# mako443/Text2Pos-CVPR2022

Hardware: AMD Instinct MI355X
Metric: cells+queries encoded/sec and top-k retrieval QPS, 256-pt cells, 12k-cell DB (higher is better)
Workload: dtype f16x3 (fp32 operands split hi+lo into fp16, 3 f16 MFMAs, fp32 accumulate; fp32-class error) for the encoders / f64 MFMA for the ranking

## Files before the change

text2pos-cvpr2022_amd/csrc/cell_encoder.hip:

```cpp
#include "../../include/t2p.h"
#include "t2p_common.h"

namespace t2p {
namespace {

struct Geo {
    int nd[3], nc[3];
    int gp;
    static constexpr int H[3] = {32, 128, 256};
    static constexpr int C[3] = {64, 128, 256};
    static constexpr int LD[3] = {96, 160, 288};
    explicit Geo(int n_pts) {
        nd[0] = n_pts;
        for (int l = 0; l < 3; l++) {
            nc[l] = (nd[l] + 1) / 2;
            if (l < 2) nd[l + 1] = nc[l];
        }
        gp = 1;
        while (gp < nc[2]) gp *= 2;
    }
    bool specialised(int l) const {
        static constexpr int ND[3] = {256, 128, 64}, NC[3] = {128, 64, 32};
        return nd[l] == ND[l] && nc[l] == NC[l];
    }
// ... 194 lines not shown
        T2P_TRY(launch_build_rows(xyz, rgb, n, cfg.n_pts, cfg.radius, gt, st));
    else if (prune_l0)
        T2P_TRY(launch_dedup_rows(xyz, rgb, n, cfg.n_pts, gt.rows[0], gt.n_rows[0], g.nc[0], st));
    return launch_sa_balance_levels(bp, Geo::H, Geo::C, st);
}

int Chunk::sa_levels(const float* xyz, const float* rgb) const {
    for (int l = 0; l < 3; l++) {
        const int H = Geo::H[l], C = Geo::C[l];
        const int cf = l == 0 ? 3 : Geo::C[l - 1];
        if (l != 0) {
            WsParams p{};
            p.A = ws.F[l - 1];
            p.lda = Geo::LD[l - 1];
            p.k_live = Geo::C[l - 1] + 4;
            p.W = W.sa_w1[l];
            p.W_x3 = f16x3() ? W.sa_w1_x3[l] : nullptr;
            p.ldw = H;
            p.bias = W.sa_b1[l];
            p.out = ws.A[l];
            p.ldo = H;
            p.relu = 0;
            p.M = n * g.nd[l];
            p.amax_out = gslot(l == 1 ? G_A2 : G_A3);
            T2P_TRY(launch_ws(WS_DENSE_STORE, Geo::LD[l - 1] - (f16x3() ? 16 : 0), H, p, st));
        }
        SaParams p{};
        p.A = ws.A[l];
        p.Bc = ws.B[l];
        p.wp = lds_btab(l) ? W.sa_w1[l] + (size_t)cf * Geo::H[l] : nullptr;
        p.W = W.sa_w2[l];
        p.W_x3 = f16x3() ? W.sa_w2_x3[l] : nullptr;
        p.bias = f16x3() ? W.sa_b2_x3[l] : W.sa_b2[l];
        p.out_scale = f16x3() ? 1.0f / W.sa_w2_scale[l] : 1.0f;
        p.out = ws.F[l];
        p.ldo = Geo::LD[l];
        p.rows = ws.gt.rows[l];
        p.n_rows = ws.gt.n_rows[l];
        p.first = ws.first;
        p.fps_idx = ws.gt.fps_idx[l];
        p.pos_src = l == 0 ? xyz : ws.F[l - 1];
        p.ld_pos = l == 0 ? 3 : Geo::LD[l - 1];
        p.pos_col0 = l == 0 ? 0 : Geo::C[l - 1];
        if (l == 0 && sa1_points()) {
            p.feat_src = rgb;
            p.w1 = W.sa_w1[0];
            p.b1 = W.sa_b1[0];
        }
        p.n_dense = g.nd[l];
        p.n_cent = g.nc[l];
        p.n_obj = n;
        p.prefix_ws = ws.prefix[l];
        p.bounds_ws = ws.bounds[l];
        p.balanced = 1;
        p.amax_out = gslot(G_F1 + l);
        if (l == 2) p.out_rows = g.gp;
        T2P_TRY(launch_ws_sa(H, C, p, st));
    }
    return 0;
}

int Chunk::global_abstraction() const {
    WsParams p{};
    p.A = ws.F[2];
    p.lda = Geo::LD[2];
    p.W = W.ga_w1;
    p.W_x3 = f16x3() ? W.ga_w1_x3 : nullptr;
    p.ldw = 512;
    p.bias = W.ga_b1;
    p.out = ws.gh;
    _Float16* gh_hi = (_Float16*)ws.gh;
    _Float16* gh_lo = gh_hi + (size_t)gh_rows(n, g) * 512;
    if (f16x3()) {
        p.out_hi = gh_hi;
        p.out_lo = gh_lo;
        p.amax_out = gslot(G_GA_H);
    }
    p.ldo = 512;
    p.relu = 1;
    p.M = n * g.gp;
    T2P_TRY(launch_ws(WS_DENSE_STORE, Geo::LD[2] - (f16x3() ? 16 : 0), 512, p, st));
    WsParams q{};
    q.A = ws.gh;
    if (f16x3()) {
        q.A_hi = gh_hi;
        q.A_lo = gh_lo;
    }
    q.lda = 512;
    q.W = W.ga_w2;
    q.W_x3 = f16x3() ? W.ga_w2_x3 : nullptr;
    q.ldw = 1024;
    q.bias = W.ga_b2;
    q.out = ws.f0;
    q.ldo = 1024;
    q.relu = 1;
    q.M = n * g.gp;
    q.group_rows = g.gp;
    return launch_ws(WS_DENSE_GROUPMAX, 512, 1024, q, st);
}

int Chunk::trunk_heads() const {
    const bool x3 = f16x3() && W.lin1_x3 && W.lin2_x3;
    const DenseW lin1{W.lin1_w, x3 ? W.lin1_x3 : nullptr, W.lin1_scale}, lin2{W.lin2_w, x3 ? W.lin2_x3 : nullptr, W.lin2_scale};
    T2P_TRY(launch_dense(ws.f0, 1024, lin1, W.lin1_b, ws.f1, 512, 0, n, 1024, 512, 1, st, nullptr, 0, gslot(G_PN_F0)));
    return launch_dense(ws.f1, 512, lin2, W.lin2_b, ws.f2, 256, 0, n, 512, 256, 1, st, nullptr, 0, gslot(G_PN_F1));
}

int Chunk::trunk(const float* xyz, const float* rgb, bool want_nbr) const {
    T2P_TRY(group(xyz, rgb, want_nbr));
    T2P_TRY(sa_levels(xyz, rgb));
    T2P_TRY(global_abstraction());
    return trunk_heads();
}

int Chunk::object_encoder(const float* center, const float* mean_rgb, int32_t o_lo, const float** emb_out) const {
    const int D = cfg.embed_dim, nfeat = n_features(cfg), ldcat = nfeat * D;
    int slot = 0;
    if (cfg.use_class && cfg.class_embed) {
        T2P_TRY(launch_gather_rownorm(W.class_embedding, cfg.class_idx + o_lo, n, D, ws.cat, ldcat, slot * D, st));
        slot++;
    } else if (cfg.use_class) {
        const float* fin = cfg.pointnet_features == 0 ? ws.f0 : (cfg.pointnet_features == 1 ? ws.f1 : ws.f2);
        const int kin = cfg.pointnet_features == 0 ? 1024 : (cfg.pointnet_features == 1 ? 512 : 256);
        const DenseW pn{W.pn_w, f16x3() ? W.pn_x3 : nullptr, W.pn_scale};
        T2P_TRY(launch_dense(fin, kin, pn, W.pn_b, ws.P, D, 0, n, kin, D, 1, st, nullptr, 0, gslot(G_PN_F0 + cfg.pointnet_features)));
        T2P_TRY(launch_rownorm(ws.P, D, n, D, ws.cat, ldcat, slot * D, st));
        slot++;
    }
    if (cfg.use_color && cfg.color_embed) {
        T2P_TRY(launch_gather_rownorm(W.color_embedding, cfg.color_idx + o_lo, n, D, ws.cat, ldcat, slot * D, st));
        slot++;
    } else if (cfg.use_color) {
        T2P_TRY(launch_mlp3_norm(mean_rgb, n, W.col_w1, W.col_b1, W.col_w2, W.col_b2, D, ws.cat, ldcat, slot * D, st));
        slot++;
    }
    if (cfg.use_position) {
        T2P_TRY(launch_mlp3_norm(center, n, W.pos_w1, W.pos_b1, W.pos_w2, W.pos_b2, D, ws.cat, ldcat, slot * D, st));
        slot++;
    }
    *emb_out = ws.cat;
    if (nfeat > 1) {
        const DenseW merge{W.merge_w, f16x3() ? W.merge_x3 : nullptr, W.merge_scale};
        T2P_TRY(launch_dense(ws.cat, ldcat, merge, W.merge_b, ws.emb, D, 0, n, ldcat, D, 1, st, nullptr, 0, gslot(G_GEMM_IN)));
        *emb_out = ws.emb;
    }
    return 0;
}

int Chunk::cell_head(const float* emb, int max_cell, float* out) const {
    const int D = cfg.embed_dim;
    T2P_TRY(launch_rownorm(emb, D, n, D, ws.embn, D, 0, st));
    const bool x3 = f16x3() && W.g_wp_x3 && W.g_wq_x3;
    const DenseW wp{W.g_wp, x3 ? W.g_wp_x3 : nullptr, W.g_wp_scale}, wq{W.g_wq, x3 ? W.g_wq_x3 : nullptr, W.g_wq_scale};
    T2P_TRY(launch_dense(ws.embn, D, wp, W.g_bp, ws.P, D, 0, n, D, D, 0, st, nullptr, 0, gslot(G_GEMM_IN)));
    T2P_TRY(launch_dense(ws.embn, D, wq, nullptr, ws.Q, D, 0, n, D, D, 0, st, nullptr, 0, gslot(G_GEMM_IN)));
    T2P_TRY(launch_knn(ws.embn, D, ws.seg_ptr, (int)nb, max_cell, cfg.knn_k, ws.knn, st));
    WsParams p{};
    p.A = ws.Q;
    p.lda = D;
    p.Bc = ws.P;
    p.W = W.g_w2;
    p.W_x3 = f16x3() ? W.g_w2_x3 : nullptr;
    p.amax_out = gslot(G_EDGE);
    p.ldw = D;
    p.bias = W.g_b2;
    p.out = ws.x1;
    p.ldo = D;
    p.relu = 1;
    p.knn_group = (n + 31) / 32 < num_cus() ? 8 : 32;
    p.n_groups = (n + p.knn_group - 1) / p.knn_group;
    p.knn_idx = ws.knn;
    p.knn_k = cfg.knn_k;
    p.n_dst = n;
    p.mean = cfg.variation == 1;
    T2P_TRY(launch_ws(WS_EDGE_KNN, D, D, p, st));
    T2P_TRY(launch_segmax(ws.x1, D, ws.seg_ptr, (int)nb, ws.pool, cfg.variation == 1, st));
    T2P_TRY(launch_gemm(ws.pool, D, W.lin_w1, W.lin_b1, ws.l1, D, 0, nb, D, D, 1, st));
    T2P_TRY(launch_gemm(ws.l1, D, W.lin_w2, W.lin_b2, ws.l2, D, 0, nb, D, D, 1, st));
    return launch_rownorm(ws.l2, D, nb, D, out, D, 0, st);
}

template <typename T>
int copy_trace(T* dst, int64_t row0, size_t width, const T* src, int64_t n, hipStream_t st) {
    if (dst == nullptr || n == 0 || width == 0) return 0;
    hipError_t e = hipMemcpyAsync(dst + row0 * width, src, (size_t)n * width * sizeof(T), hipMemcpyDeviceToDevice, st);
    if (e != hipSuccess) {
        set_error("encode_cells: trace copy failed: %s", hipGetErrorString(e));
        return (int)e;
    }
    return 0;
}

int Chunk::copy_traces(const t2p_cell_trace& tr, int64_t obj0, bool trunk_ran, const float* emb) const {
    for (int l = 0; trunk_ran && l < 3; l++) {
        T2P_TRY(copy_trace(tr.fps_idx[l], obj0, g.nc[l], ws.gt.fps_idx[l], n, st));
        T2P_TRY(copy_trace(tr.nbr[l], obj0, (size_t)g.nc[l] * 32, ws.gt.nbr[l], n, st));
        T2P_TRY(copy_trace(tr.cnt[l], obj0, g.nc[l], ws.gt.cnt[l], n, st));
        if (tr.sa_out[l] && n > 0) {
            const int rows = l == 2 ? g.gp : g.nc[l];
            const size_t ld = Geo::LD[l] * sizeof(float);
            hipError_t e = hipSuccess;
            if (rows == g.nc[l])
                e = hipMemcpy2DAsync(tr.sa_out[l] + obj0 * g.nc[l] * Geo::LD[l], ld, ws.F[l], ld, (Geo::C[l] + 4) * sizeof(float),
                                     (size_t)n * g.nc[l], hipMemcpyDeviceToDevice, st);
            for (int cc = 0; rows != g.nc[l] && cc < g.nc[l] && e == hipSuccess; cc++)
                e = hipMemcpy2DAsync(tr.sa_out[l] + (obj0 * g.nc[l] + cc) * Geo::LD[l], g.nc[l] * ld, ws.F[l] + (size_t)cc * Geo::LD[l],
                                     rows * ld, (Geo::C[l] + 4) * sizeof(float), (size_t)n, hipMemcpyDeviceToDevice, st);
            if (e != hipSuccess) {
                set_error("encode_cells: trace copy failed: %s", hipGetErrorString(e));
                return (int)e;
            }
        }
    }
    if (trunk_ran) {
        T2P_TRY(copy_trace(tr.features0, obj0, 1024, ws.f0, n, st));
        T2P_TRY(copy_trace(tr.features1, obj0, 512, ws.f1, n, st));
        T2P_TRY(copy_trace(tr.features2, obj0, 256, ws.f2, n, st));
    }
    if (emb != nullptr) {
        T2P_TRY(copy_trace(tr.obj_emb, obj0, cfg.embed_dim, emb, n, st));
        T2P_TRY(copy_trace(tr.knn_idx, obj0, cfg.knn_k, ws.knn, n, st));
    }
    return 0;
}

int64_t next_chunk_end(const int32_t* cp, int64_t c0, int64_t n_cells, int chunk) {
    int64_t c1 = c0 + 1;
    while (c1 < n_cells && (cp[c1 + 1] - cp[c0]) <= chunk) c1++;
    return c1;
}

int fill_group_tables(const char* what, GroupTables& gt, int n_pts, int self_loops, int share_mask, uint8_t* const* fps_idx,
                      uint16_t* const* rows, uint16_t* const* n_rows, uint8_t* const* nbr, uint8_t* const* cnt) {
    const Geo g(n_pts);
    gt = GroupTables{};
    gt.self_loops = self_loops ? 1 : 0;
    for (int l = 0; l < 3; l++) {
        if (rows) T2P_CHECK_ARG(fps_idx[l] && rows[l] && n_rows[l], "%s: NULL table of level %d", what, l);
        gt.fps_idx[l] = fps_idx[l];
        gt.rows[l] = rows ? rows[l] : nullptr;
        gt.n_rows[l] = rows ? n_rows[l] : nullptr;
        gt.nbr[l] = nbr ? nbr[l] : nullptr;
        gt.cnt[l] = cnt ? cnt[l] : nullptr;
        gt.n_dense[l] = g.nd[l];
        gt.n_cent[l] = g.nc[l];
        gt.share_tail[l] = (share_mask >> l) & 1;
    }
    return 0;
}

int group_rows(const char* what, const float* xyz, int64_t n_obj, int32_t n_pts, const float* radius_host, int32_t self_loops,
               int32_t share_mask, uint8_t* const* fps_idx, uint16_t* const* rows, uint16_t* const* n_rows, t2p_stream_t stream) {
    T2P_CHECK_ARG(xyz && radius_host && fps_idx && rows && n_rows, "%s: NULL argument", what);
    T2P_CHECK_ARG((share_mask & ~2) == 0, "%s: share_mask=%#x (bit 1: SA level 2; no other level has a shared form)", what, share_mask);
    T2P_CHECK_ARG(share_mask == 0 || n_pts == 256, "%s: shared lists exist for 256 points per object (n_pts = %d)", what, n_pts);
    GroupTables gt;
    T2P_TRY(fill_group_tables(what, gt, n_pts, self_loops, share_mask, fps_idx, rows, n_rows, nullptr, nullptr));
    return launch_sample_group(xyz, n_obj, n_pts, radius_host, gt, (hipStream_t)stream);
}

int group_rows_built(const char* what, const float* xyz, const float* rgb, int64_t n_obj, int32_t n_pts, const float* radius_host,
                     int32_t self_loops, int32_t share_mask, int prune_dup, uint8_t* const* fps_idx, uint16_t* const* rows,
                     uint16_t* const* n_rows, t2p_stream_t stream) {
    T2P_CHECK_ARG(xyz && rgb && radius_host && fps_idx && rows && n_rows, "%s: NULL argument", what);
    T2P_CHECK_ARG(n_obj >= 0, "%s: negative size", what);
    T2P_CHECK_ARG((share_mask & ~2) == 0, "%s: share_mask=%#x (bit 1: SA level 2; no other level has a shared form)", what, share_mask);
    T2P_CHECK_ARG(n_pts == 256, "%s: built for 256 points per object (n_pts = %d)", what, n_pts);
    GroupTables gt;
    T2P_TRY(fill_group_tables(what, gt, n_pts, self_loops, share_mask, fps_idx, rows, n_rows, nullptr, nullptr));
    gt.mask_l0 = 1;
    gt.prune_dup[1] = gt.prune_dup[2] = prune_dup;
    T2P_CHECK_ARG((((uintptr_t)xyz | (uintptr_t)rgb | (uintptr_t)rows[0] | (uintptr_t)rows[1] | (uintptr_t)rows[2]) & 15) == 0,
                  "%s: xyz, rgb and rows must be 16-byte aligned", what);
    T2P_TRY(launch_sample_group(xyz, n_obj, n_pts, radius_host, gt, (hipStream_t)stream));
    return launch_build_rows(xyz, rgb, n_obj, n_pts, radius_host, gt, (hipStream_t)stream);
}

}
}

using namespace t2p;

extern "C" {

size_t t2p_encode_cells_workspace_bytes(int64_t n_obj, int64_t n_cells, const t2p_cell_config* cfg) {
    if (cfg == nullptr || n_obj <= 0) return 256;
    int64_t n = default_chunk(*cfg);
    if (n > n_obj) n = n_obj;
    int64_t nb = n_cells < n ? n_cells : n;
    Bump b{nullptr, 0, 0};
    return carve_cells(b, n, nb > 0 ? nb : 1, *cfg, nullptr) + 256;
}

int t2p_encode_cells(const float* xyz, const float* rgb, const float* center, const float* mean_rgb,
                     const int32_t* cell_ptr_host, const int32_t* cell_ptr, int64_t n_obj, int64_t n_cells,
                     const t2p_cell_weights* w, const t2p_cell_config* cfg, float* out, const t2p_cell_trace* trace,
                     void* workspace, size_t workspace_bytes, t2p_stream_t stream) {
    hipStream_t st = (hipStream_t)stream;
    T2P_TRY(check_cfg(cfg));
    T2P_CHECK_ARG(w != nullptr && cell_ptr_host != nullptr && cell_ptr != nullptr, "encode_cells: NULL argument");
    T2P_CHECK_ARG(n_cells >= 0 && n_obj >= 0, "encode_cells: negative size");
    if (n_cells == 0) return 0;
    if (cfg->objects_only)
        T2P_CHECK_ARG(trace != nullptr && trace->obj_emb != nullptr, "encode_cells: objects_only needs trace->obj_emb");
    else
        T2P_CHECK_ARG(out != nullptr, "encode_cells: out is NULL");
    T2P_CHECK_ARG(!cfg->class_embed || w->class_embedding != nullptr, "encode_cells: class_embedding weights missing");
    T2P_CHECK_ARG(!cfg->color_embed || w->color_embedding != nullptr, "encode_cells: color_embedding weights missing");
// ... 140 lines not shown
```

text2pos-cvpr2022_amd/csrc/t2p_common.h:

```cpp
#pragma once
#include <hip/hip_runtime.h>
#include <stdint.h>
#include <stdio.h>

namespace t2p {

void set_error(const char* fmt, ...);

#define T2P_E_ARG (-1)
#define T2P_E_WORKSPACE (-2)
#define T2P_E_UNSUPPORTED (-3)

#define T2P_CHECK_ARG(cond, ...)                  \
    do {                                          \
        if (!(cond)) {                            \
            ::t2p::set_error(__VA_ARGS__);        \
            return T2P_E_ARG;                     \
        }                                         \
    } while (0)

#define T2P_CHECK_LAUNCH(name)                                                   \
    do {                                                                         \
        hipError_t e__ = hipGetLastError();                                      \
        if (e__ != hipSuccess) {                                                 \
// ... 39 lines not shown
    return lo;
}
__device__ __forceinline__ void lds_barrier() { asm volatile("s_waitcnt lgkmcnt(0)\n\ts_barrier" ::: "memory"); }
typedef double f64x4 __attribute__((ext_vector_type(4)));

int num_cus();
int matrix_wgs();
int reserve_lds(const void* kernel, size_t bytes, const char* what);

inline size_t align_up(size_t v, size_t a) { return (v + a - 1) / a * a; }
struct Bump {
    char* base;
    size_t off, cap;
    template <typename T>
    T* take(size_t n) {
        off = align_up(off, 256);
        T* p = (T*)(base ? base + off : nullptr);
        off += n * sizeof(T);
        return p;
    }
};

enum GuardSlot {
    G_INPUT = 0,
    G_A2 = 2, G_A3 = 4,
    G_F1 = 6, G_F2 = 7, G_F3 = 8,
    G_GEMM_IN = 9,
    G_GA_H = 10, G_PN_F0 = 11, G_PN_F1 = 12, G_PN_F2 = 13, G_EDGE = 14,
    G_SLOTS = 16
};
struct GuardBounds {
    float wp_l1[3];
    float a1_l1;
    float a1_bmax;
    float ga1_l1;
    float ga1_bmax;
};
constexpr float kGuardFloor = 16384.f;
constexpr float kGuardTiny = 0.0078125f;
#ifdef __HIPCC__
__device__ __forceinline__ void guard_publish_above(uint32_t* slot, float m, float floor_) {
    if (slot == nullptr) return;
    if (!__any(m > floor_)) return;
#pragma unroll
    for (int o = 32; o > 0; o >>= 1) m = fmaxf(m, __shfl_xor(m, o, 64));
    if ((threadIdx.x & 63) == 0) atomicMax(slot, __float_as_uint(m));
}
__device__ __forceinline__ void guard_publish_bits_above(uint32_t* slot, uint32_t bits, uint32_t floor_bits) {
    if (slot == nullptr) return;
    if (!__any(bits > floor_bits)) return;
#pragma unroll
    for (int o = 32; o > 0; o >>= 1) {
        const uint32_t other = (uint32_t)__shfl_xor((int)bits, o, 64);
        bits = other > bits ? other : bits;
    }
    if ((threadIdx.x & 63) == 0) atomicMax(slot, bits);
}
__device__ __forceinline__ void guard_publish_exact(uint32_t* slot, float m) {
    if (slot == nullptr) return;
#pragma unroll
    for (int o = 32; o > 0; o >>= 1) m = fmaxf(m, __shfl_xor(m, o, 64));
    if ((threadIdx.x & 63) == 0) {
        const uint32_t b = __float_as_uint(m);
        if (b > __atomic_load_n(slot, __ATOMIC_RELAXED)) atomicMax(slot, b);
    }
}
__device__ __forceinline__ void guard_track_bits(uint32_t& acc, int lane_bits ) {
#pragma unroll
    for (int o = 32; o > 0; o >>= 1) {
        const int other = __shfl_xor(lane_bits, o, 64);
        lane_bits = other > lane_bits ? other : lane_bits;
    }
    const uint32_t b = (uint32_t)__builtin_amdgcn_readfirstlane(lane_bits);
    acc = b > acc ? b : acc;
}
#endif
int launch_guard_check(const uint32_t* guard, int32_t* overflow_flag, const GuardBounds& b, hipStream_t st);

struct ProfScope {
    ProfScope(const char* name, hipStream_t st);
    ~ProfScope();
    int slot;
    hipStream_t st;
    void* ev_end;
    int reps;
};
#define T2P_REPEAT(ps) for (int rep_ = (ps).reps; rep_ > 0; --rep_)

struct GroupTables {
    uint8_t* fps_idx[3];
    uint8_t* nbr[3];
    uint8_t* cnt[3];
    uint16_t* rows[3];
    uint16_t* n_rows[3];
    int self_loops;
    int share_tail[3];
    int prune_dup[3];
    int mask_l0;
    int n_dense[3];
    int n_cent[3];
    float* B[3];
    const float* wp[3];
    int H[3];
    float* tail[3];
    int ld_tail[3], tail_col0[3];
    int tail_rows[3];
    float* A1;
    const float* w1;
    const float* b1;
    const float* rgb;
    int H1;
    uint32_t* guard;
};
int launch_sample_group(const float* xyz, int64_t n_obj, int n_pts, const float radius[3], GroupTables gt,
                        hipStream_t st);
int launch_dedup_rows(const float* xyz, const float* rgb, int64_t n_obj, int n_pts, uint16_t* rows, uint16_t* n_rows,
                      int n_cent, hipStream_t st);
int launch_build_rows(const float* xyz, const float* rgb, int64_t n_obj, int n_pts, const float radius[3], const GroupTables& gt,
                      hipStream_t st);

int launch_rownorm(const float* in, int ld_in, int64_t n_rows, int dim, float* out, int ld_out, int col0,
                   hipStream_t st);
int launch_gather_rownorm(const float* table, const int32_t* idx, int64_t n_rows, int dim, float* out, int ld_out,
                          int col0, hipStream_t st);
int launch_segmax(const float* in, int dim, const int32_t* seg_ptr, int n_seg, float* out, int mean,
                  hipStream_t st);
int launch_knn(const float* x, int dim, const int32_t* seg_ptr, int n_seg, int max_seg_rows, int k,
               int32_t* out_idx, hipStream_t st);
int launch_mlp3_norm(const float* in3, int64_t n_rows, const float* w1, const float* b1, const float* w2,
                     const float* b2, int D, float* out, int ld_out, int col0, hipStream_t st);
int launch_pack_objects(const float* raw_xyz, const float* raw_rgb, const int32_t* obj_ptr, const int32_t* sample_idx,
                        const float* rot, int64_t n_obj, int n_pts, float* xyz, float* rgb, float* center, float* mean_rgb,
                        hipStream_t st);
int launch_pack_scene(const float* raw_xyz, const float* raw_rgb, const int32_t* obj_ptr, const int32_t* obj_id, const uint64_t* key,
                      const float* scene_center, const float* scene_color, int64_t n_out, int n_pts, float* xyz, float* rgb,
                      float* center, float* mean_rgb, int32_t* idx_out, hipStream_t st);
int launch_pack_scene_aug(const float* raw_xyz, const float* raw_rgb, const float* raw_mirror_xy, const int32_t* obj_ptr,
                          const int32_t* obj_id, const uint64_t* key, const uint8_t* flip, const float* rot, const float* scene_center,
                          const float* center_mirror_xy, const float* scene_color, int64_t n_out, int n_pts, float* xyz, float* rgb,
                          float* center, float* mean_rgb, int32_t* idx_out, hipStream_t st);
int launch_pairwise_ranking(const float* scores, int batch, float margin, float* row_loss, float* d_scores, float* row_cnt,
                            hipStream_t st);
int launch_hardest_ranking(const float* scores, int batch, float margin, float* best, int32_t* where, float* d_scores,
                           hipStream_t st);
int launch_cell_index(const int32_t* cell_ptr, int n_cells, int32_t o_lo, int32_t* seg_ptr_local, int32_t* first,
                      hipStream_t st, uint32_t* guard_to_clear = nullptr);

int launch_gemm(const float* A, int lda, const float* W, const float* bias, float* C, int ldc, int c0, int64_t M,
                int K, int N, int relu, hipStream_t st, const float* resid = nullptr, int ldr = 0);
int launch_gemm_skinny(const float* A, int lda, const float* W, float* C, int ldc, int64_t M, int K, int N, hipStream_t st);
int launch_gemm_x3(const float* A, int lda, const void* Wx, float scale, const float* bias, float* C, int ldc, int c0,
                   int64_t M, int K, int N, int relu, hipStream_t st, const float* resid = nullptr, int ldr = 0,
                   uint32_t* amax_in = nullptr );
struct DenseW { const float* w; const void* x3; float scale; };
inline int launch_dense(const float* A, int lda, const DenseW& W, const float* bias, float* C, int ldc, int c0, int64_t M, int K, int N,
                        int relu, hipStream_t st, const float* resid = nullptr, int ldr = 0, uint32_t* amax_in = nullptr) {
    if (W.x3 != nullptr) return launch_gemm_x3(A, lda, W.x3, W.scale, bias, C, ldc, c0, M, K, N, relu, st, resid, ldr, amax_in);
    return launch_gemm(A, lda, W.w, bias, C, ldc, c0, M, K, N, relu, st, resid, ldr);
}

size_t gemm_tn_workspace_bytes(int64_t M, int K1, int N);
int launch_edge_counts(const uint16_t* rows, const uint16_t* n_rows, const int32_t* first_obj, int64_t n_obj, int n_dense, int n_cent,
                       int self_loops, int32_t* counts, hipStream_t st);
int launch_edge_expand(const uint16_t* rows, const uint16_t* n_rows, const int32_t* first_obj, const int32_t* cent_ptr, int64_t n_obj,
                       int n_dense, int n_cent, int self_loops, int32_t* src, int32_t* dst, hipStream_t st);
size_t linear_wgrad_workspace_bytes(int64_t M, int K1, int N);
int launch_linear_wgrad_f32(const float* dY, int lda, const float* X, int ldb, float* dW, int ldc, float* colsum, int64_t M, int K1, int N,
                            void* ws, size_t ws_bytes, hipStream_t st);
int launch_gemm_tn(const float* A, int lda, const float* B, int ldb, float* C, int ldc, int64_t M, int K1, int N, void* ws,
                   size_t ws_bytes, hipStream_t st);

enum WsMode { WS_DENSE_STORE = 0, WS_DENSE_GROUPMAX = 1, WS_EDGE_KNN = 3 };
struct WsParams {
    const float* A;
    int lda;
    int k_live;
    const float* Bc;
    const float* W;
    int ldw;
    const void* W_x3;
    const void* A_hi;
    const void* A_lo;
    void* out_hi;
    void* out_lo;
    const float* bias;
    float* out;
    int ldo;
    int relu;
    int64_t n_groups;
    int64_t M;
    uint32_t* amax_out;
    const int32_t* knn_idx;
    int knn_k;
    int64_t n_dst;
    int mean;
    int knn_group;
    int group_rows;
};
int launch_ws(int mode, int K, int N, const WsParams& p, hipStream_t st);

struct SaParams {
    const float* A;
    const float* Bc;
    const float* wp;
    const float* W;
    const void* W_x3;
    const float* bias;
    float out_scale;
    float* out;
    int ldo;
    const uint16_t* rows;
    const uint16_t* n_rows;
    const int32_t* first;
    const uint8_t* fps_idx;
    const float* pos_src;
    int ld_pos, pos_col0;
    const float* feat_src;
    const float* w1;
    const float* b1;
    int n_dense, n_cent;
    int64_t n_obj;
    int32_t* prefix_ws;
    int32_t* bounds_ws;
    int balanced;
    uint32_t* amax_out;
    int out_rows;
};
int launch_ws_sa(int H, int C, const SaParams& p, hipStream_t st);
int launch_sa_balance(const SaParams& p, int tile_rows, int n_wg, hipStream_t st);
int launch_sa_balance_arrays(const uint16_t* n_rows, int n, int tile_rows, int n_wg, int32_t* prefix, int32_t* bounds, hipStream_t st);
constexpr int kSaTailCode = 64;
bool sa_rows_selected(int H, int C, const SaParams& p);
int launch_sa_rows(int H, int C, const SaParams& p, hipStream_t st);
int sa_rows_launch_shape(int64_t n_obj, int* tile_rows, int* n_wg);
bool sa_points_selected(int H, int C, const SaParams& p);
int launch_sa_points(int H, int C, const SaParams& p, hipStream_t st);
int sa_points_launch_shape(int64_t n_obj, int* tile_rows, int* n_wg);
bool sa3_selected(int H, int C, const SaParams& p);
int launch_sa3(const SaParams& p, hipStream_t st);
int sa3_launch_shape(int64_t n_obj, int* tile_rows, int* n_wg);
inline bool sa_shares_tail_rows(int l, int H, int C, const SaParams& p, int n_pts, int tuning) {
    return l == 1 && n_pts == 256 && !(tuning & 4) && p.n_dense == 128 && p.n_cent == 64 && sa_rows_selected(H, C, p);
}
int launch_sa_balance_levels(const SaParams p[3], const int H[3], const int C[3], hipStream_t st);

int launch_bilstm_impl(const float* gate_table , const float* whh ,
                       const void* whh_x3 ,
                       float whh_scale, const int32_t* tokens , const int32_t* lengths, int B, int T, int V, int D,
                       float* hdir_ws , float* out ,
                       hipStream_t st);

int launch_lstm_cell_fwd(const float* pre, const float* table, const int32_t* tokens, const int32_t* lengths, int64_t B, int T,
                         int D, int step, int reverse, const float* c_prev, const float* h_prev, float* gates, float* c,
                         float* h, hipStream_t st);
int launch_lstm_cell_bwd(const float* dh_gemm, const float* dh_carry_in, const float* dc_in, const float* gates,
                         const float* c_prev, const float* c, const int32_t* lengths, int64_t B, int D, int step, float* d_pre,
                         float* dc_out, float* dh_carry_out, hipStream_t st);

size_t bn_train_workspace_bytes(int64_t rows, int n_seg, int C);
int launch_bn_relu_train_forward(const float* x, const int32_t* seg_ptr, int n_seg, int64_t rows, int C, const float* gamma,
                                 const float* beta, float eps, int relu, float* y, float* mean, float* invstd,
                                 float* var_unbiased, double* part, hipStream_t st);
int launch_bn_relu_train_backward(const float* dy, const float* x, const float* beta, const int32_t* seg_ptr, int n_seg,
                                  int64_t rows, int C, const float* mean, const float* invstd, const float* gamma, int relu,
                                  float* dx, float* dgamma_seg, float* dbeta_seg, double* part, hipStream_t st);
int launch_edge_feat_fwd(const float* x, const float* pos, const float* pos_c, const int32_t* src, const int32_t* dst, int64_t E,
                         int C, int W, float* out, hipStream_t st);
int launch_edge_feat_bwd(const float* dout, const int32_t* src, int64_t E, int C, int W, float* dx, hipStream_t st);
int launch_pair_feat_fwd(const float* x, const int32_t* tgt, const int32_t* src, int64_t E, int D, float* out, hipStream_t st);
int launch_pair_feat_bwd(const float* dout, const int32_t* tgt, const int32_t* src, int64_t E, int D, float* dx, hipStream_t st);
int launch_segment_mean(const float* x, const int32_t* seg_ptr, int n_seg, int C, float* out, hipStream_t st);
int launch_segment_mean_backward(const float* dout, const int32_t* seg_ptr, int n_seg, int C, float* dx, hipStream_t st);
int launch_rownorm_bwd(const float* x, const float* dy, int64_t n_rows, int dim, float* dx, hipStream_t st);
int launch_segment_max(const float* x, const int32_t* seg_ptr, int n_seg, int C, float* out, int32_t* arg, hipStream_t st);
int launch_segment_max_backward(const float* dout, const int32_t* arg, const int32_t* seg_ptr, int n_seg, int C, float* dx,
                                hipStream_t st);

int launch_classifier_heads(const float* f2, const float* w, const float* bias, int64_t n, int C1, int C2, float* class_pred,
                            float* color_pred, hipStream_t st);
int launch_softmax_xent(const float* logits, int ld, const int32_t* labels, int64_t n, int C, float* row_loss, float* d_logits,
                        int ldd, int32_t* correct, hipStream_t st);
int launch_one_cell_index(int64_t n, int32_t* seg_ptr_local, int32_t* first, hipStream_t st, uint32_t* guard_to_clear);

size_t sim_topk_workspace_bytes(int64_t nq, int64_t nc, int k);
int launch_sim_topk(const float* Q, const float* C, int64_t nq, int64_t nc, int dim, int k, int64_t c_index_offset,
                    int64_t* out_idx, double* out_score, void* ws, size_t ws_bytes, hipStream_t st);
int launch_sim_topk_grouped(const float* Q, const float* C, const int32_t* query_group, const int32_t* cell_group, int64_t nq,
                            int64_t nc, int dim, int k, int64_t c_index_offset, int64_t* out_idx, double* out_score, void* ws,
                            size_t ws_bytes, hipStream_t st);

}
```

text2pos-cvpr2022_amd/csrc/tg_gemm_x3.hip:

```cpp
#include "t2p_common.h"

namespace t2p {
namespace {


constexpr int BK = 32;
constexpr int LDT = BK + 8;
template <int TS>
struct X3Cfg {
    static constexpr int PLANE = TS * LDT;
    static constexpr size_t kLds = (size_t)2  * 2  * 2  * PLANE * sizeof(_Float16);
    static constexpr int TPR = 256 / TS;
    static constexpr int KPT = BK / TPR;
    static constexpr int MI = TS / 64;
};

template <int TS>
__global__ __launch_bounds__(256, 2) void k_gemm_x3(const float* __restrict__ A, int lda, const _Float16* __restrict__ Wx,
                                                    int kp , float inv_scale,
                                                    const float* __restrict__ bias, float* C, int ldc, int c0, int64_t M,
                                                    int K, int N, int relu, const float* R, int ldr, uint32_t* amax_in) {
    using Cf = X3Cfg<TS>;
    constexpr int BM = TS, BN = TS, PLANE = Cf::PLANE, KPT = Cf::KPT, MI = Cf::MI;
    extern __shared__ __attribute__((aligned(16))) _Float16 sm[];
    const int tid = threadIdx.x, lane = tid & 63, wave = tid >> 6;
    const int wr = wave >> 1, wc = wave & 1, h = lane >> 5, l31 = lane & 31;
    const int64_t m0 = (int64_t)blockIdx.x * BM;
    const int n0 = blockIdx.y * BN;
    const _Float16* Whi = Wx;
    const _Float16* Wlo = Wx + (size_t)N * kp;

    const int s_row = tid / Cf::TPR, s_k = (tid % Cf::TPR) * KPT;
    const bool a_ok = (m0 + s_row) < M;
    const bool w_ok = (n0 + s_row) < N;
    const float* a_ptr = A + (m0 + s_row) * (int64_t)lda + s_k;
    const _Float16* wh_ptr = Whi + (size_t)(n0 + s_row) * kp + s_k;
    const _Float16* wl_ptr = Wlo + (size_t)(n0 + s_row) * kp + s_k;
    f32x4 ra[KPT / 4];
    uint4 rwh[KPT / 8], rwl[KPT / 8];
    float gmax = 0.f;

    auto load_tile = [&](int k0) {
#pragma unroll
        for (int i = 0; i < KPT / 4; i++) {
            const int k = k0 + s_k + 4 * i;
            ra[i] = (a_ok && k < K) ? *(const f32x4*)(a_ptr + k0 + 4 * i) : f32x4{0.f, 0.f, 0.f, 0.f};
        }
#pragma unroll
        for (int i = 0; i < KPT / 8; i++) {
            rwh[i] = w_ok ? *(const uint4*)(wh_ptr + k0 + 8 * i) : uint4{0, 0, 0, 0};
            rwl[i] = w_ok ? *(const uint4*)(wl_ptr + k0 + 8 * i) : uint4{0, 0, 0, 0};
        }
    };
    auto store_tile = [&](int buf) {
        _Float16* base = sm + (size_t)buf * 4 * PLANE;
#pragma unroll
        for (int i = 0; i < KPT / 4; i++) {
            const f32x4 v = ra[i];
            gmax = fmaxf(fmaxf(gmax, fmaxf(fabsf(v[0]), fabsf(v[1]))), fmaxf(fabsf(v[2]), fabsf(v[3])));
            const fp16x2 h01 = cvt_pk_f16(v[0], v[1]), h23 = cvt_pk_f16(v[2], v[3]);
            const fp16x2 l01 = cvt_pk_f16(sub_half<0>(v[0], h01), sub_half<1>(v[1], h01));
            const fp16x2 l23 = cvt_pk_f16(sub_half<0>(v[2], h23), sub_half<1>(v[3], h23));
            uint2 ph, pl;
            ph.x = __builtin_bit_cast(uint32_t, h01); ph.y = __builtin_bit_cast(uint32_t, h23);
            pl.x = __builtin_bit_cast(uint32_t, l01); pl.y = __builtin_bit_cast(uint32_t, l23);
            *(uint2*)(base + s_row * LDT + s_k + 4 * i) = ph;
            *(uint2*)(base + PLANE + s_row * LDT + s_k + 4 * i) = pl;
        }
#pragma unroll
        for (int i = 0; i < KPT / 8; i++) {
            *(uint4*)(base + 2 * PLANE + s_row * LDT + s_k + 8 * i) = rwh[i];
            *(uint4*)(base + 3 * PLANE + s_row * LDT + s_k + 8 * i) = rwl[i];
        }
    };

    f32x16 acc[MI][MI];
#pragma unroll
    for (int i = 0; i < MI; i++)
#pragma unroll
        for (int j = 0; j < MI; j++)
#pragma unroll
            for (int e = 0; e < 16; e++) acc[i][j][e] = 0.f;

    load_tile(0);
    store_tile(0);
    __syncthreads();
    int buf = 0;
    for (int k0 = 0; k0 < K; k0 += BK, buf ^= 1) {
        const bool more = k0 + BK < K;
        if (more) load_tile(k0 + BK);
        const _Float16* base = sm + (size_t)buf * 4 * PLANE;
#pragma unroll
        for (int ks = 0; ks < BK / 16; ks++) {
            half8 a_hi[MI], a_lo[MI], b_hi[MI], b_lo[MI];
#pragma unroll
            for (int i = 0; i < MI; i++) {
                const _Float16* p = base + (wr * (TS / 2) + i * 32 + l31) * LDT + ks * 16 + h * 8;
                a_hi[i] = *(const half8*)p;
                a_lo[i] = *(const half8*)(p + PLANE);
                const _Float16* q = base + 2 * PLANE + (wc * (TS / 2) + i * 32 + l31) * LDT + ks * 16 + h * 8;
                b_hi[i] = *(const half8*)q;
                b_lo[i] = *(const half8*)(q + PLANE);
            }
#pragma unroll
            for (int i = 0; i < MI; i++)
#pragma unroll
                for (int j = 0; j < MI; j++) {
                    acc[i][j] = __builtin_amdgcn_mfma_f32_32x32x16_f16(a_hi[i], b_hi[j], acc[i][j], 0, 0, 0);
                    acc[i][j] = __builtin_amdgcn_mfma_f32_32x32x16_f16(a_hi[i], b_lo[j], acc[i][j], 0, 0, 0);
                    acc[i][j] = __builtin_amdgcn_mfma_f32_32x32x16_f16(a_lo[i], b_hi[j], acc[i][j], 0, 0, 0);
                }
        }
        if (more) store_tile(buf ^ 1);
        __syncthreads();
    }

    if (blockIdx.y == 0) guard_publish_exact(amax_in, gmax);
#pragma unroll
    for (int j = 0; j < MI; j++) {
        const int col = n0 + wc * (TS / 2) + j * 32 + l31;
        if (col >= N) continue;
        const float bv = bias ? bias[col] : 0.f;
#pragma unroll
        for (int i = 0; i < MI; i++) {
#pragma unroll
            for (int e = 0; e < 16; e++) {
                const int64_t row = m0 + wr * (TS / 2) + i * 32 + (e & 3) + 8 * (e >> 2) + 4 * h;
                if (row < M) {
                    float v = fmaf(acc[i][j][e], inv_scale, bv);
                    if (relu) v = v <= 0.f ? 0.f : v;
                    if (R) v += R[row * (int64_t)ldr + col];
                    C[row * (int64_t)ldc + c0 + col] = v;
                }
            }
        }
    }
}

}

int launch_gemm_x3(const float* A, int lda, const void* Wx, float scale, const float* bias, float* C, int ldc, int c0,
                   int64_t M, int K, int N, int relu, hipStream_t st, const float* resid, int ldr, uint32_t* amax_in) {
    T2P_CHECK_ARG(K % 4 == 0 && N % 8 == 0 && lda % 4 == 0 && scale > 0.f, "gemm_x3: K=%d %% 4, N=%d %% 8, lda=%d %% 4", K, N, lda);
    T2P_CHECK_ARG((((uintptr_t)A) & 15) == 0 && (((uintptr_t)Wx) & 15) == 0, "gemm_x3: A and W must be 16-byte aligned");
    if (M == 0) return 0;
    const int kp = (K + 31) / 32 * 32;
    ProfScope ps_("tg_gemm_x3", st);
    const int64_t tiles128 = ((M + 127) / 128) * ((N + 127) / 128);
    if (tiles128 * 2 <= num_cus()) {
        T2P_TRY(reserve_lds((const void*)k_gemm_x3<64>, X3Cfg<64>::kLds, "gemm_x3"));
        dim3 grid((unsigned)((M + 63) / 64), (unsigned)((N + 63) / 64));
        hipLaunchKernelGGL(k_gemm_x3<64>, grid, dim3(256), X3Cfg<64>::kLds, st, A, lda, (const _Float16*)Wx, kp, 1.0f / scale, bias, C, ldc,
                           c0, M, K, N, relu, resid, ldr, amax_in);
    } else {
        T2P_TRY(reserve_lds((const void*)k_gemm_x3<128>, X3Cfg<128>::kLds, "gemm_x3"));
        dim3 grid((unsigned)((M + 127) / 128), (unsigned)((N + 127) / 128));
        hipLaunchKernelGGL(k_gemm_x3<128>, grid, dim3(256), X3Cfg<128>::kLds, st, A, lda, (const _Float16*)Wx, kp, 1.0f / scale, bias, C, ldc,
                           c0, M, K, N, relu, resid, ldr, amax_in);
    }
    T2P_CHECK_LAUNCH("gemm_x3");
    return 0;
}

}
```

Measured before the change: 160,500.

## Fuse P/Q projection GEMMs into one panel-ordered x3 kernel with register prefetch

Adds a 128x128 f16x3 GEMM kernel that takes two output weight sets and covers both with one grid. It walks the grid in groups of 8 row panels so that nearby blocks share the same A rows in cache, and prefetches the next two K tiles into registers while the current tile is multiplied. The cell head now issues the P and Q projections as a single launch over the shared normalized embeddings, and the single-output large case also goes through this kernel. This removes one launch and repeated A traffic, but adds register pressure from the two-stage register buffers, and the generic path's performance changes too.

```diff
diff --git a/text2pos-cvpr2022_amd/csrc/cell_encoder.hip b/text2pos-cvpr2022_amd/csrc/cell_encoder.hip
--- a/text2pos-cvpr2022_amd/csrc/cell_encoder.hip
+++ b/text2pos-cvpr2022_amd/csrc/cell_encoder.hip
@@ -370,8 +370,13 @@
     T2P_TRY(launch_rownorm(emb, D, n, D, ws.embn, D, 0, st));
     const bool x3 = f16x3() && W.g_wp_x3 && W.g_wq_x3;
     const DenseW wp{W.g_wp, x3 ? W.g_wp_x3 : nullptr, W.g_wp_scale}, wq{W.g_wq, x3 ? W.g_wq_x3 : nullptr, W.g_wq_scale};
-    T2P_TRY(launch_dense(ws.embn, D, wp, W.g_bp, ws.P, D, 0, n, D, D, 0, st, nullptr, 0, gslot(G_GEMM_IN)));
-    T2P_TRY(launch_dense(ws.embn, D, wq, nullptr, ws.Q, D, 0, n, D, D, 0, st, nullptr, 0, gslot(G_GEMM_IN)));
+    if (x3) {
+        T2P_TRY(launch_gemm_x3_pair(ws.embn, D, wp.x3, wp.scale, W.g_bp, ws.P, wq.x3, wq.scale, nullptr, ws.Q, D, 0, n, D, D, 0, st,
+                                    gslot(G_GEMM_IN)));
+    } else {
+        T2P_TRY(launch_dense(ws.embn, D, wp, W.g_bp, ws.P, D, 0, n, D, D, 0, st, nullptr, 0, gslot(G_GEMM_IN)));
+        T2P_TRY(launch_dense(ws.embn, D, wq, nullptr, ws.Q, D, 0, n, D, D, 0, st, nullptr, 0, gslot(G_GEMM_IN)));
+    }
     T2P_TRY(launch_knn(ws.embn, D, ws.seg_ptr, (int)nb, max_cell, cfg.knn_k, ws.knn, st));
     WsParams p{};
     p.A = ws.Q;
diff --git a/text2pos-cvpr2022_amd/csrc/t2p_common.h b/text2pos-cvpr2022_amd/csrc/t2p_common.h
--- a/text2pos-cvpr2022_amd/csrc/t2p_common.h
+++ b/text2pos-cvpr2022_amd/csrc/t2p_common.h
@@ -215,6 +215,9 @@
 int launch_gemm_x3(const float* A, int lda, const void* Wx, float scale, const float* bias, float* C, int ldc, int c0,
                    int64_t M, int K, int N, int relu, hipStream_t st, const float* resid = nullptr, int ldr = 0,
                    uint32_t* amax_in = nullptr );
+int launch_gemm_x3_pair(const float* A, int lda, const void* Wx1, float scale1, const float* bias1, float* C1, const void* Wx2,
+                        float scale2, const float* bias2, float* C2, int ldc, int c0, int64_t M, int K, int N, int relu, hipStream_t st,
+                        uint32_t* amax_in = nullptr);
 struct DenseW { const float* w; const void* x3; float scale; };
 inline int launch_dense(const float* A, int lda, const DenseW& W, const float* bias, float* C, int ldc, int c0, int64_t M, int K, int N,
                         int relu, hipStream_t st, const float* resid = nullptr, int ldr = 0, uint32_t* amax_in = nullptr) {
diff --git a/text2pos-cvpr2022_amd/csrc/tg_gemm_x3.hip b/text2pos-cvpr2022_amd/csrc/tg_gemm_x3.hip
--- a/text2pos-cvpr2022_amd/csrc/tg_gemm_x3.hip
+++ b/text2pos-cvpr2022_amd/csrc/tg_gemm_x3.hip
@@ -137,6 +137,194 @@
     }
 }
 
+struct X3Out {
+    const _Float16* Wx;
+    float inv_scale;
+    const float* bias;
+    float* C;
+};
+struct X3Regs {
+    f32x4 ra[4];
+    uint4 rwh[2], rwl[2];
+};
+#ifndef T2P_X3_ABL
+#define T2P_X3_ABL 0
+#endif
+
+__global__ __launch_bounds__(256, 2) void k_gemm_x3_panels(const float* __restrict__ A, int lda, int kp, X3Out o0, X3Out o1, int nb1,
+                                                           int nbt , int np , int ldc,
+                                                           int c0, int64_t M, int K, int N, int relu, const float* R, int ldr,
+                                                           uint32_t* amax_in) {
+    using Cf = X3Cfg<128>;
+    constexpr int TS = 128, PLANE = Cf::PLANE, MI = Cf::MI;
+    static_assert(MI == 2 && BK == 32, "the staging maps and X3Regs are written for the 128 x 128 x 32 tile");
+    extern __shared__ __attribute__((aligned(16))) _Float16 sm[];
+    const int tid = threadIdx.x, lane = tid & 63, wave = tid >> 6;
+    const int wr = wave >> 1, wc = wave & 1, h = lane >> 5, l31 = lane & 31;
+
+    const int lin = blockIdx.x;
+    const int np8 = (T2P_X3_ABL & 1) ? 0 : (np & ~7);
+    int panel, cb;
+    if (lin < np8 * nbt) {
+        const int g = lin / (8 * nbt), l = lin - g * 8 * nbt;
+        panel = g * 8 + (l & 7);
+        cb = l >> 3;
+    } else {
+        const int l = lin - np8 * nbt;
+        panel = np8 + l / nbt;
+        cb = l % nbt;
+    }
+    const bool second = cb >= nb1;
+    const X3Out o = second ? o1 : o0;
+    const int64_t m0 = (int64_t)panel * TS;
+    const int n0 = (second ? cb - nb1 : cb) * TS;
+    const _Float16* Whi = o.Wx;
+    const _Float16* Wlo = o.Wx + (size_t)N * kp;
+
+    const int a_r = wave * 32 + (lane >> 3), a_kc = (lane & 7) * 4;
+    const int w_r = wave * 32 + (lane >> 2), w_kc = (lane & 3) * 8;
+    const float* a_ptr[4];
+    size_t w_off[2];
+#pragma unroll
+    for (int i = 0; i < 4; i++) a_ptr[i] = A + min(m0 + a_r + 8 * i, M - 1) * (int64_t)lda;
+#pragma unroll
+    for (int i = 0; i < 2; i++) w_off[i] = (size_t)min(n0 + w_r + 16 * i, N - 1) * kp + w_kc;
+    float gmax = 0.f;
+
+    auto load_tile = [&](X3Regs& r, int k0) {
+#pragma unroll
+        for (int i = 0; i < 4; i++) r.ra[i] = *(const f32x4*)(a_ptr[i] + min(k0 + a_kc, K - 4));
+#pragma unroll
+        for (int i = 0; i < 2; i++) {
+            r.rwh[i] = *(const uint4*)(Whi + w_off[i] + k0);
+            r.rwl[i] = *(const uint4*)(Wlo + w_off[i] + k0);
+        }
+    };
+    auto store_tile = [&](const X3Regs& r, int buf, int k0, bool mask ) {
+        _Float16* base = sm + (size_t)buf * 4 * PLANE;
+        const bool zero = mask && k0 + a_kc >= K;
+#pragma unroll
+        for (int i = 0; i < 4; i++) {
+            const f32x4 v = zero ? f32x4{0.f, 0.f, 0.f, 0.f} : r.ra[i];
+            gmax = fmaxf(fmaxf(gmax, fmaxf(fabsf(v[0]), fabsf(v[1]))), fmaxf(fabsf(v[2]), fabsf(v[3])));
+            const fp16x2 h01 = cvt_pk_f16(v[0], v[1]), h23 = cvt_pk_f16(v[2], v[3]);
+            const fp16x2 l01 = cvt_pk_f16(sub_half<0>(v[0], h01), sub_half<1>(v[1], h01));
+            const fp16x2 l23 = cvt_pk_f16(sub_half<0>(v[2], h23), sub_half<1>(v[3], h23));
+            uint2 ph, pl;
+            ph.x = __builtin_bit_cast(uint32_t, h01); ph.y = __builtin_bit_cast(uint32_t, h23);
+            pl.x = __builtin_bit_cast(uint32_t, l01); pl.y = __builtin_bit_cast(uint32_t, l23);
+            *(uint2*)(base + (a_r + 8 * i) * LDT + a_kc) = ph;
+            *(uint2*)(base + PLANE + (a_r + 8 * i) * LDT + a_kc) = pl;
+        }
+#pragma unroll
+        for (int i = 0; i < 2; i++) {
+            *(uint4*)(base + 2 * PLANE + (w_r + 16 * i) * LDT + w_kc) = r.rwh[i];
+            *(uint4*)(base + 3 * PLANE + (w_r + 16 * i) * LDT + w_kc) = r.rwl[i];
+        }
+    };
+
+    f32x16 acc[MI][MI];
+#pragma unroll
+    for (int i = 0; i < MI; i++)
+#pragma unroll
+        for (int j = 0; j < MI; j++)
+#pragma unroll
+            for (int e = 0; e < 16; e++) acc[i][j][e] = 0.f;
+
+    auto mma_k16 = [&](int buf, int ks) {
+        const _Float16* base = sm + (size_t)buf * 4 * PLANE;
+        half8 a_hi[MI], a_lo[MI], b_hi[MI], b_lo[MI];
+#pragma unroll
+        for (int i = 0; i < MI; i++) {
+            const _Float16* p = base + (wr * (TS / 2) + i * 32 + l31) * LDT + ks * 16 + h * 8;
+            a_hi[i] = *(const half8*)p;
+            a_lo[i] = *(const half8*)(p + PLANE);
+            const _Float16* q = base + 2 * PLANE + (wc * (TS / 2) + i * 32 + l31) * LDT + ks * 16 + h * 8;
+            b_hi[i] = *(const half8*)q;
+            b_lo[i] = *(const half8*)(q + PLANE);
+        }
+#pragma unroll
+        for (int i = 0; i < MI; i++)
+#pragma unroll
+            for (int j = 0; j < MI; j++) {
+                acc[i][j] = __builtin_amdgcn_mfma_f32_32x32x16_f16(a_hi[i], b_hi[j], acc[i][j], 0, 0, 0);
+                acc[i][j] = __builtin_amdgcn_mfma_f32_32x32x16_f16(a_hi[i], b_lo[j], acc[i][j], 0, 0, 0);
+                acc[i][j] = __builtin_amdgcn_mfma_f32_32x32x16_f16(a_lo[i], b_hi[j], acc[i][j], 0, 0, 0);
+            }
+    };
+    auto mma_tile = [&](int buf) {
+        __builtin_amdgcn_sched_barrier(0);
+        mma_k16(buf, 0);
+        __builtin_amdgcn_sched_barrier(0);
+        mma_k16(buf, 1);
+    };
+
+    const int nk = (K + BK - 1) / BK;
+    X3Regs r0, r1;
+    if (nk > 0) {
+        load_tile(r0, 0);
+        if (nk > 1) load_tile(r1, BK);
+        store_tile(r0, 0, 0, true);
+        __syncthreads();
+        int t = 0;
+        for (; t + 3 < nk; t += 2) {
+            load_tile(r0, (t + 2) * BK);
+            mma_tile(0);
+            store_tile(r1, 1, (t + 1) * BK, false);
+            __syncthreads();
+            load_tile(r1, (t + 3) * BK);
+            mma_tile(1);
+            store_tile(r0, 0, (t + 2) * BK, false);
+            __syncthreads();
+        }
+        const int rem = nk - t;
+        if (rem == 3) load_tile(r0, (t + 2) * BK);
+        mma_tile(0);
+        if (rem >= 2) {
+            store_tile(r1, 1, (t + 1) * BK, true);
+            __syncthreads();
+            mma_tile(1);
+            if (rem == 3) {
+                store_tile(r0, 0, (t + 2) * BK, true);
+                __syncthreads();
+                mma_tile(0);
+            }
+        }
+    }
+
+    if (cb == 0) guard_publish_exact(amax_in, gmax);
+#pragma unroll
+    for (int j = 0; j < MI; j++) {
+        const int col = n0 + wc * (TS / 2) + j * 32 + l31;
+        if (col >= N) continue;
+        const float bv = o.bias ? o.bias[col] : 0.f;
+#pragma unroll
+        for (int i = 0; i < MI; i++) {
+#pragma unroll
+            for (int e = 0; e < 16; e++) {
+                const int64_t row = m0 + wr * (TS / 2) + i * 32 + (e & 3) + 8 * (e >> 2) + 4 * h;
+                if (row < M) {
+                    float v = fmaf(acc[i][j][e], o.inv_scale, bv);
+                    if (relu) v = v <= 0.f ? 0.f : v;
+                    if (R) v += R[row * (int64_t)ldr + col];
+                    o.C[row * (int64_t)ldc + c0 + col] = v;
+                }
+            }
+        }
+    }
+}
+
+int launch_panels(const float* A, int lda, int kp, const X3Out* o, int n_out, int ldc, int c0, int64_t M, int K, int N, int relu,
+                  hipStream_t st, const float* resid, int ldr, uint32_t* amax_in) {
+    const int64_t np = (M + 127) / 128;
+    const int nb1 = (N + 127) / 128, nbt = n_out * nb1;
+    T2P_CHECK_ARG(np * nbt < (1LL << 31), "gemm_x3: %lld x %d tiles exceed the grid", (long long)np, nbt);
+    T2P_TRY(reserve_lds((const void*)k_gemm_x3_panels, X3Cfg<128>::kLds, "gemm_x3"));
+    hipLaunchKernelGGL(k_gemm_x3_panels, dim3((unsigned)(np * nbt)), dim3(256), X3Cfg<128>::kLds, st, A, lda, kp, o[0], o[n_out - 1], nb1,
+                       nbt, (int)np, ldc, c0, M, K, N, relu, resid, ldr, amax_in);
+    return 0;
+}
+
 }
 
 int launch_gemm_x3(const float* A, int lda, const void* Wx, float scale, const float* bias, float* C, int ldc, int c0,
@@ -153,13 +341,30 @@
         hipLaunchKernelGGL(k_gemm_x3<64>, grid, dim3(256), X3Cfg<64>::kLds, st, A, lda, (const _Float16*)Wx, kp, 1.0f / scale, bias, C, ldc,
                            c0, M, K, N, relu, resid, ldr, amax_in);
     } else {
-        T2P_TRY(reserve_lds((const void*)k_gemm_x3<128>, X3Cfg<128>::kLds, "gemm_x3"));
-        dim3 grid((unsigned)((M + 127) / 128), (unsigned)((N + 127) / 128));
-        hipLaunchKernelGGL(k_gemm_x3<128>, grid, dim3(256), X3Cfg<128>::kLds, st, A, lda, (const _Float16*)Wx, kp, 1.0f / scale, bias, C, ldc,
-                           c0, M, K, N, relu, resid, ldr, amax_in);
+        const X3Out o{(const _Float16*)Wx, 1.0f / scale, bias, C};
+        T2P_TRY(launch_panels(A, lda, kp, &o, 1, ldc, c0, M, K, N, relu, st, resid, ldr, amax_in));
     }
     T2P_CHECK_LAUNCH("gemm_x3");
     return 0;
 }
 
-}
+int launch_gemm_x3_pair(const float* A, int lda, const void* Wx1, float scale1, const float* bias1, float* C1, const void* Wx2,
+                        float scale2, const float* bias2, float* C2, int ldc, int c0, int64_t M, int K, int N, int relu, hipStream_t st,
+                        uint32_t* amax_in) {
+    const int64_t tiles128 = ((M + 127) / 128) * ((N + 127) / 128);
+    if (M == 0 || tiles128 * 2 <= num_cus()) {
+        T2P_TRY(launch_gemm_x3(A, lda, Wx1, scale1, bias1, C1, ldc, c0, M, K, N, relu, st, nullptr, 0, amax_in));
+        return launch_gemm_x3(A, lda, Wx2, scale2, bias2, C2, ldc, c0, M, K, N, relu, st, nullptr, 0, amax_in);
+    }
+    T2P_CHECK_ARG(K % 4 == 0 && N % 8 == 0 && lda % 4 == 0 && scale1 > 0.f && scale2 > 0.f, "gemm_x3: K=%d %% 4, N=%d %% 8, lda=%d %% 4", K,
+                  N, lda);
+    T2P_CHECK_ARG((((uintptr_t)A) & 15) == 0 && (((uintptr_t)Wx1) & 15) == 0 && (((uintptr_t)Wx2) & 15) == 0,
+                  "gemm_x3: A and W must be 16-byte aligned");
+    ProfScope ps_("tg_gemm_x3", st);
+    const X3Out o[2] = {{(const _Float16*)Wx1, 1.0f / scale1, bias1, C1}, {(const _Float16*)Wx2, 1.0f / scale2, bias2, C2}};
+    T2P_TRY(launch_panels(A, lda, (K + 31) / 32 * 32, o, 2, ldc, c0, M, K, N, relu, st, nullptr, 0, amax_in));
+    T2P_CHECK_LAUNCH("gemm_x3");
+    return 0;
+}
+
+}
```

Result: no change. 161,400, median of 6 (+0.6%).
